# PierfrancescoArdino/C2M

Hardware: AMD Instinct MI355X
Metric: generator train-step frames/sec at 128x256x7 (higher is better)
Workload: dtype f32; 1 GPU; BASELINE configs[1]: 128x256, 7-frame clips (2 in + 5 predicted), batch 8/GPU, fp32, generator fwd+bwd only (no D), VGG loss on, random-init weights; global_batch=8, parallelism=single

## Files before the change

c2m_amd/csrc/conv_igemm.hip:

```cpp
#include "common.h"
#include "dtype.h"
#include <stdlib.h>
#include <string.h>
#include "conv_store.h"

typedef float f32x16 __attribute__((ext_vector_type(16)));
typedef float f32x4 __attribute__((ext_vector_type(4)));

struct ConvP {
    const float* A;
    const float* X;
    float* Y;
    const float* bias;
    const int4* ktab;
    int M, nk, lda;
    int Npix, To, Ho, Wo;
    int Ti, Hi, Wi;
    int st, sh, sw;
    int in_sc;
    long in_sn, in_st, in_sh;
    long out_sn, out_sc, out_st, out_sh, out_sw, out_off;
    long slab_stride;
    unsigned x_bytes;
    float* Y2;
// ... 935 lines not shown
        if (chunk < chunk_end) PB_CHUNK(s1);
    }
#undef PB_CHUNK
#undef PB_TAP

    const bool direct = blk.nz == 1;
    const bool yh = p.yh && direct;
    float* __restrict__ Yb = p.Y + (long)blk.z * p.slab_stride;
    if (yh && !p.Y2 && p.out_sw == 1 && (p.Wo & 7) == 0 && (p.out_off & 7) == 0 && (p.out_sc & 7) == 0 && (p.out_sn & 7) == 0 &&
        (p.out_st & 7) == 0 && (p.out_sh & 7) == 0 && ((uintptr_t)p.Y & 15) == 0 && BM >= 64) {
        float* __restrict__ T = reinterpret_cast<float*>(&sA[0][0]) + wave * (64 * 64);
        bf16_t* __restrict__ yimg = reinterpret_cast<bf16_t*>(p.Y) + p.out_off + (long)n_img * p.out_sn + (long)t_img * p.out_st;
#pragma unroll
        for (int h = 0; h < MI / 2; ++h) {
#pragma unroll
            for (int q = 0; q < 2; ++q)
#pragma unroll
                for (int jj = 0; jj < NI; ++jj)
#pragma unroll
                    for (int r = 0; r < 16; ++r) {
                        const int cl = q * 32 + (r & 3) + 8 * (r >> 2) + 4 * (lane >> 5);
                        float v = acc[2 * h + q][jj][r];
                        const int row = m0 + h * 64 + cl;
                        if (p.bias && row < p.M) v += p.bias[row];
                        T[cl * 64 + jj * 32 + (lane & 31)] = c2m_act(v, p.act, p.slope);
                    }
#pragma unroll
            for (int it = 0; it < 8; ++it) {
                const int cl = it * 8 + (lane >> 3), px = (lane & 7) * 8;
                const float4 v0 = *reinterpret_cast<const float4*>(&T[cl * 64 + px]);
                const float4 v1 = *reinterpret_cast<const float4*>(&T[cl * 64 + px + 4]);
                const int row = m0 + h * 64 + cl;
                const int oy = oy0 + wave * NI + (px >> 5), ox = ox0 + (px & 31);
                if (row < p.M && oy < p.Ho && ox < p.Wo) {
                    const bf16x8 o = {(bf16_t)v0.x, (bf16_t)v0.y, (bf16_t)v0.z, (bf16_t)v0.w,
                                      (bf16_t)v1.x, (bf16_t)v1.y, (bf16_t)v1.z, (bf16_t)v1.w};
                    __builtin_nontemporal_store(o, reinterpret_cast<bf16x8*>(yimg + (long)row * p.out_sc + (long)oy * p.out_sh + ox));
                }
            }
        }
        return;
    }
    if (!yh && !p.Y2 && p.out_sw == 1 && (p.Wo & 3) == 0 && (p.out_off & 3) == 0 && (p.out_sc & 3) == 0 && (p.out_sn & 3) == 0 &&
        (p.slab_stride & 3) == 0 && ((uintptr_t)p.Y & 15) == 0 && BM >= 64) {
        float* __restrict__ T = reinterpret_cast<float*>(&sA[0][0]) + wave * (64 * 64);
        float* __restrict__ yimg = Yb + p.out_off + (long)n_img * p.out_sn + (long)t_img * p.out_st;
#pragma unroll
        for (int h = 0; h < MI / 2; ++h) {
#pragma unroll
            for (int q = 0; q < 2; ++q)
#pragma unroll
                for (int jj = 0; jj < NI; ++jj)
#pragma unroll
                    for (int r = 0; r < 16; ++r) {
                        const int cl = q * 32 + (r & 3) + 8 * (r >> 2) + 4 * (lane >> 5);
                        float v = acc[2 * h + q][jj][r];
                        if (direct) {
                            const int row = m0 + h * 64 + cl;
                            if (p.bias && row < p.M) v += p.bias[row];
                            v = c2m_act(v, p.act, p.slope);
                        }
                        T[cl * 64 + jj * 32 + (lane & 31)] = v;
                    }
#pragma unroll
            for (int it = 0; it < 16; ++it) {
                const int cl = it * 4 + (lane >> 4), px = (lane & 15) * 4;
                const float4 v = *reinterpret_cast<const float4*>(&T[cl * 64 + px]);
                const int row = m0 + h * 64 + cl;
                const int oy = oy0 + wave * NI + (px >> 5), ox = ox0 + (px & 31);
                if (row < p.M && oy < p.Ho && ox < p.Wo) {
                    f32x4 vv = {v.x, v.y, v.z, v.w};
                    __builtin_nontemporal_store(vv, reinterpret_cast<f32x4*>(yimg + (long)row * p.out_sc + (long)oy * p.out_sh + ox));
                }
            }
        }
        return;
    }
#pragma unroll
    for (int j = 0; j < NI; ++j) {
        const int oy = oy0 + wave * NI + j, ox = ox0 + (lane & 31);
        if (oy >= p.Ho || ox >= p.Wo) continue;
        float* ybase = Yb;
        long yidx = p.out_off + (long)n_img * p.out_sn + (long)t_img * p.out_st + (long)oy * p.out_sh + (long)ox * p.out_sw;
        long row_stride = p.out_sc;
        if (p.Y2) {
            const int tp = t_img * p.ps_t + p.po_t - p.lo_t, yp = oy * p.ps_y + p.po_y - p.lo_y,
                      xp = ox * p.ps_x + p.po_x - p.lo_x;
            if ((unsigned)tp < (unsigned)p.ext_t && (unsigned)yp < (unsigned)p.ext_y && (unsigned)xp < (unsigned)p.ext_x) {
                ybase = p.Y2;
                yidx = (long)n_img * p.y2_sn + (long)tp * p.y2_st + (long)yp * p.y2_sh + xp;
                row_stride = p.y2_sc;
            }
        }
#pragma unroll
        for (int i = 0; i < MI; ++i)
#pragma unroll
            for (int r = 0; r < 16; ++r) {
                const int row = m0 + i * 32 + (r & 3) + 8 * (r >> 2) + 4 * (lane >> 5);
                if (row < p.M) {
                    float v = acc[i][j][r];
                    if (direct) {
                        if (p.bias) v += p.bias[row];
                        v = c2m_act(v, p.act, p.slope);
                    }
                    if (yh) reinterpret_cast<bf16_t*>(ybase)[yidx + (long)row * row_stride] = (bf16_t)v;
                    else ybase[yidx + (long)row * row_stride] = v;
                }
            }
    }
}

template <int BM>
static int launch_patch_bf16(const ConvP& p, int splits, hipStream_t s) {
    const long tiles = (long)(p.Npix / (p.Ho * p.Wo)) * ((p.Ho + 7) / 8) * ((p.Wo + 31) / 32);
    dim3 grid((unsigned)(tiles * c2m_cdiv(p.M, BM) * splits));
    hipLaunchKernelGGL((conv_patch3x3_bf16_kernel<BM>), grid, dim3(256), 0, s, p);
    return (int)hipGetLastError();
}

template <class T>
__global__ void splitk_reduce_kernel(const float* __restrict__ slab, T* __restrict__ out,
                                     const float* __restrict__ bias, long total, int S, long chan_stride, int M, int act,
                                     float slope) {
    for (long i = blockIdx.x * (long)blockDim.x + threadIdx.x; i < total; i += (long)gridDim.x * blockDim.x) {
        float acc = 0.f;
        for (int z = 0; z < S; ++z) acc += slab[(long)z * total + i];
        if (bias) acc += bias[(int)((i / chan_stride) % M)];
        c2m_st(out, i, c2m_act(acc, act, slope));
    }
}

template <typename I, class T = float>
__global__ void splitk_reduce_vec_kernel(const float4* __restrict__ slab, T* __restrict__ out,
                                         const float* __restrict__ bias, long total4_, int S, long chan_stride4_, int M,
                                         int act, float slope) {
    const I total4 = (I)total4_, chan_stride4 = (I)chan_stride4_;
    for (I i = blockIdx.x * (I)blockDim.x + threadIdx.x; i < total4; i += (I)gridDim.x * blockDim.x) {
        float4 acc = make_float4(0.f, 0.f, 0.f, 0.f);
        for (int z = 0; z < S; ++z) {
            const float4 v = slab[(long)z * total4_ + i];
            acc.x += v.x; acc.y += v.y; acc.z += v.z; acc.w += v.w;
        }
        if (bias) {
            const float b = bias[(int)((i / chan_stride4) % (I)M)];
            acc.x += b; acc.y += b; acc.z += b; acc.w += b;
        }
        c2m_st4(out + 4 * (long)i, make_float4(c2m_act(acc.x, act, slope), c2m_act(acc.y, act, slope), c2m_act(acc.z, act, slope),
                                               c2m_act(acc.w, act, slope)));
    }
}

template <int NS> static int launch_thin_fwd(const ConvP& p, hipStream_t s);
template <int KW> static int launch_thin_rows(const ConvP& p, int ns, int ntg, int Cin, int xdesc, hipStream_t s);

#ifndef C2M_IGEMM_U
#define C2M_IGEMM_U 1
#endif
#ifndef C2M_BF16_U
#define C2M_BF16_U 2
#endif

template <int BM, int BN, int WGM, int WGN>
static int launch_igemm(const ConvP& p, int ns, int splits, hipStream_t s, bool bf16) {
    dim3 grid((unsigned)c2m_cdiv(p.Npix, BN) * c2m_cdiv(p.M, BM) * splits * p.ncls);
    constexpr int U = (BM == 128) ? C2M_IGEMM_U : 1;
    if (bf16) {
        constexpr int UB = C2M_BF16_U;
        switch (ns) {
            case 1: hipLaunchKernelGGL((conv_igemm_kernel<BM, BN, WGM, WGN, 1, UB, true>), grid, dim3(256), 0, s, p); break;
            case 2: hipLaunchKernelGGL((conv_igemm_kernel<BM, BN, WGM, WGN, 2, UB, true>), grid, dim3(256), 0, s, p); break;
            case 4: hipLaunchKernelGGL((conv_igemm_kernel<BM, BN, WGM, WGN, 4, UB, true>), grid, dim3(256), 0, s, p); break;
            default: return (int)hipErrorInvalidValue;
        }
        return (int)hipGetLastError();
    }
    switch (ns) {
        case 1: hipLaunchKernelGGL((conv_igemm_kernel<BM, BN, WGM, WGN, 1, U>), grid, dim3(256), 0, s, p); break;
        case 2: hipLaunchKernelGGL((conv_igemm_kernel<BM, BN, WGM, WGN, 2, 1>), grid, dim3(256), 0, s, p); break;
        case 4: hipLaunchKernelGGL((conv_igemm_kernel<BM, BN, WGM, WGN, 4, 1>), grid, dim3(256), 0, s, p); break;
        default: return (int)hipErrorInvalidValue;
    }
    return (int)hipGetLastError();
}

static void igemm_tile(int M, int& BM, int& BN) {
    if (M <= 32) { BM = 32; BN = 256; }
    else if (M <= 64) { BM = 64; BN = 128; }
    else { BM = 128; BN = 128; }
}

C2M_API int c2m_conv_igemm_splits(int M, int nk, int Npix) {
    int BM, BN;
    igemm_tile(M, BM, BN);
    const long tiles = (long)c2m_cdiv(M, BM) * c2m_cdiv(Npix, BN);
#ifndef C2M_SPLIT_TARGET
#define C2M_SPLIT_TARGET 1280
#endif
    if (tiles >= 768 || nk < 8) return 1;
    long S = (C2M_SPLIT_TARGET + tiles - 1) / tiles;
    if (S > nk / 4) S = nk / 4;
    if (S > 128) S = 128;
    if (S < 2) return 1;
    const int per = c2m_cdiv(nk, (int)S);
    return c2m_cdiv(nk, per);
}

C2M_API int c2m_conv_igemm(const float* A, const void* X, void* Y, void* Y_interior, const float* bias,
                           const int* ktab, const int64_t* g, int act, float slope, void* stream) {
    C2M_ENTER();
    ConvP p;
    p.A = A; p.X = (const float*)X; p.Y = (float*)Y; p.bias = bias; p.ktab = reinterpret_cast<const int4*>(ktab);
    p.Y2 = (float*)Y_interior;
    p.ps_t = (int)g[C2M_G_PS_T]; p.ps_y = (int)g[C2M_G_PS_Y]; p.ps_x = (int)g[C2M_G_PS_X]; p.po_t = (int)g[C2M_G_PO_T]; p.po_y = (int)g[C2M_G_PO_Y];
    p.po_x = (int)g[C2M_G_PO_X]; p.lo_t = (int)g[C2M_G_LO_T]; p.lo_y = (int)g[C2M_G_LO_Y]; p.lo_x = (int)g[C2M_G_LO_X]; p.ext_t = (int)g[C2M_G_EXT_T];
    p.ext_y = (int)g[C2M_G_EXT_Y]; p.ext_x = (int)g[C2M_G_EXT_X]; p.y2_sn = g[C2M_G_Y2_SN]; p.y2_sc = g[C2M_G_Y2_SC]; p.y2_st = g[C2M_G_Y2_ST]; p.y2_sh = g[C2M_G_Y2_SH];
    p.M = (int)g[C2M_G_M]; p.nk = (int)g[C2M_G_NK]; p.lda = (int)g[C2M_G_LDA];
    p.Npix = (int)g[C2M_G_NPIX]; p.To = (int)g[C2M_G_TO]; p.Ho = (int)g[C2M_G_HO]; p.Wo = (int)g[C2M_G_WO];
    p.Ti = (int)g[C2M_G_TI]; p.Hi = (int)g[C2M_G_HI]; p.Wi = (int)g[C2M_G_WI];
    p.st = (int)g[C2M_G_ST]; p.sh = (int)g[C2M_G_SH]; p.sw = (int)g[C2M_G_SW];
    p.in_sn = g[C2M_G_IN_SN]; p.in_st = g[C2M_G_IN_ST]; p.in_sh = g[C2M_G_IN_SH];
    p.out_sn = g[C2M_G_OUT_SN]; p.out_sc = g[C2M_G_OUT_SC]; p.out_st = g[C2M_G_OUT_ST]; p.out_sh = g[C2M_G_OUT_SH]; p.out_sw = g[C2M_G_OUT_SW]; p.out_off = g[C2M_G_OUT_OFF];
    p.reflect = (int)g[C2M_G_REFLECT]; p.is3d = (int)g[C2M_G_IS3D];
    const int ns = (int)g[C2M_G_NS];
    p.in_sc = (int)g[C2M_G_IN_SC];
    const int splits = (int)g[C2M_G_SPLITS];
    p.slab_stride = g[C2M_G_SLAB_STRIDE];
    if (g[C2M_G_X_BYTES] <= 0 || g[C2M_G_X_BYTES] >= 0x80000000LL) return (int)hipErrorInvalidValue;
    p.x_bytes = (unsigned)g[C2M_G_X_BYTES];
    p.act = act; p.slope = slope;
    p.xh = (int)g[C2M_G_X_TYPE]; p.yh = (int)g[C2M_G_Y_TYPE];
    if ((p.xh | p.yh) & ~1) return (int)hipErrorInvalidValue;
    if (p.M <= 0 || p.Npix <= 0) return 0;
    if (p.nk <= 0 || (p.lda & 3) || (((uintptr_t)A) & 15) || splits < 1) return (int)hipErrorInvalidValue;
    if (p.Y2 && splits != 1) return (int)hipErrorInvalidValue;
    p.ksteps_per_split = c2m_cdiv(p.nk, splits);
    if (!g[C2M_G_PATCH] && c2m_cdiv(p.nk, p.ksteps_per_split) != splits) return (int)hipErrorInvalidValue;
    p.splits = splits;
    p.ncls = g[C2M_G_NCLS] > 1 ? (int)g[C2M_G_NCLS] : 1;
    if (p.ncls > 8) return (int)hipErrorInvalidValue;
    p.a_cls = g[C2M_G_A_CLS]; p.ktab_cls = (int)g[C2M_G_KTAB_CLS];
    p.out_off_c[0] = p.out_off; p.po_c[0][0] = p.po_t; p.po_c[0][1] = p.po_y; p.po_c[0][2] = p.po_x;
    for (int c = 0; c < p.ncls && p.ncls > 1; ++c) {
        p.out_off_c[c] = g[C2M_G_CLS_OUT_OFF + c];
        for (int d = 0; d < 3; ++d) p.po_c[c][d] = (int)g[C2M_G_CLS_PO + 3 * c + d];
    }
    if (p.ncls > 1 && (g[C2M_G_PATCH] || (p.a_cls & 3))) return (int)hipErrorInvalidValue;
    hipStream_t s = (hipStream_t)stream;
    if (g[C2M_G_G8] == 1) {
        const int C = (int)g[C2M_G_CIN], taps = (int)g[C2M_G_TAPS];
        if (g[C2M_G_PRECISION] != 1 || !p.xh || g[C2M_G_PATCH] || C <= 0 || taps <= 0 || taps > 64 || (((uintptr_t)A | (uintptr_t)X) & 15))
            return (int)hipErrorInvalidValue;
        p.g8_nch = c2m_cdiv(C, 16); p.g8_ntaps = taps; p.g8_CB = c2m_cdiv(C, 8); p.g8_Mpad = c2m_cdiv(p.M, 128) * 128;
        if (p.nk != taps * p.g8_nch || p.in_st != (long)p.Hi * p.Wi || p.in_sh != p.Wi) return (int)hipErrorInvalidValue;
        const long plane = (long)p.Ti * p.Hi * p.Wi * 16, ab = (long)p.nk * 2 * p.g8_Mpad * 16;
        if (plane * p.g8_CB > (long)p.x_bytes || p.x_bytes % (plane * p.g8_CB) || ab * p.ncls >= 0x80000000LL)
            return (int)hipErrorInvalidValue;
        p.g8_plane_bytes = (unsigned)plane; p.g8_a_bytes = (unsigned)ab;
        const unsigned ptiles = (unsigned)c2m_cdiv(p.Npix, 256);
        int v = (int)g[C2M_G_G8_VARIANT] & 255;
        p.g8_dbg = (int)(g[C2M_G_G8_VARIANT] >> 8);
        if (v == 0) v = p.M <= 32 ? 1 : ((p.M <= 64 || (p.M % 128 >= 1 && p.M % 128 <= 64)) ? 5 : 3);
#define G8_LAUNCH(BM, UU, NB, WG) do {                                                                                     \
            dim3 grid(ptiles * (unsigned)c2m_cdiv(p.M, BM) * (unsigned)(splits * p.ncls));                                  \
            hipLaunchKernelGGL((conv_gather_nc8_kernel<BM, UU, NB, WG>), grid, dim3(256), 0, s, p); } while (0)
        switch (v) {
            case 1: G8_LAUNCH(32, 4, 2, 2); break;
            case 2: G8_LAUNCH(64, 2, 3, 2); break;
            case 3: G8_LAUNCH(128, 2, 3, 2); break;
            case 4: G8_LAUNCH(64, 1, 4, 3); break;
            case 5: G8_LAUNCH(64, 2, 2, 3); break;
            case 6: G8_LAUNCH(128, 1, 4, 2); break;
            case 7: G8_LAUNCH(32, 2, 3, 2); break;
            default: return (int)hipErrorInvalidValue;
        }
#undef G8_LAUNCH
        return (int)hipGetLastError();
    }
    if (g[C2M_G_PATCH]) {
        if (ns != 1 || p.st != 1 || p.sh != 1 || p.sw != 1) return (int)hipErrorInvalidValue;
        p.iy0 = (int)g[C2M_G_PATCH_IY0]; p.ix0 = (int)g[C2M_G_PATCH_IX0];
        for (int i = 0; i < 3; ++i) { p.pty[i] = (int)g[C2M_G_PATCH_TY + i]; p.ptx[i] = (int)g[C2M_G_PATCH_TX + i]; }
        p.nchunks = p.nk / 9;
        p.cin = (int)g[C2M_G_CIN];
        if (p.nchunks * 9 != p.nk || p.cin <= 0 || p.cin > p.nchunks * 16) return (int)hipErrorInvalidValue;
        p.ksteps_per_split = c2m_cdiv(p.nchunks, splits);
        if (c2m_cdiv(p.nchunks, p.ksteps_per_split) != splits) return (int)hipErrorInvalidValue;
        if (g[C2M_G_PRECISION] == 1) {
            if (p.lda % 128 != 0 || p.lda < p.M || !p.xh) return (int)hipErrorInvalidValue;
            if (p.M <= 32)      return launch_patch_bf16<32>(p, splits, s);
            else if (p.M <= 64 || p.cin <= 256) return launch_patch_bf16<64>(p, splits, s);
            else                return launch_patch_bf16<128>(p, splits, s);
        }
        if (p.xh || p.yh) return (int)hipErrorInvalidValue;
        if (p.M <= 32)      return launch_patch<32, 256, 1, 4>(p, splits, s);
        else if (p.M <= 64) return launch_patch<64, 128, 2, 2>(p, splits, s);
        else                return launch_patch<128, 128, 2, 2>(p, splits, s);
    }
    if (p.M <= 4 && splits == 1 && p.Npix >= 16384 && !p.Y2 && p.ncls == 1) {
        if (p.xh || p.yh) return (int)hipErrorInvalidValue;
        const int kw = (int)(g[C2M_G_SQUARE_KW] < 0 ? -g[C2M_G_SQUARE_KW] : g[C2M_G_SQUARE_KW]);
        if (p.M <= 3 && (kw == 3 || kw == 7) && !p.is3d && p.To == 1 && p.st == 1 && p.sh == 1 && p.sw == 1 && p.Wo % 4 == 0 &&
            g[C2M_G_TAPS] == kw * kw && g[C2M_G_CIN] > 0 && g[C2M_G_CIN] * kw * kw * 16 <= 48 * 1024) {
            if (kw == 3) return launch_thin_rows<3>(p, ns, (int)g[C2M_G_NTG], (int)g[C2M_G_CIN], g[C2M_G_SQUARE_KW] < 0, s);
            return launch_thin_rows<7>(p, ns, (int)g[C2M_G_NTG], (int)g[C2M_G_CIN], g[C2M_G_SQUARE_KW] < 0, s);
        }
        if (ns == 1) return launch_thin_fwd<1>(p, s);
        if (ns == 2) return launch_thin_fwd<2>(p, s);
        return launch_thin_fwd<4>(p, s);
    }
    const bool bf16 = g[C2M_G_PRECISION] == 1;
    if (bf16 ? !p.xh : (p.xh || p.yh)) return (int)hipErrorInvalidValue;
    if (p.M <= 32)      return launch_igemm<32, 256, 1, 4>(p, ns, splits, s, bf16);
    else if (p.M <= 64) return launch_igemm<64, 128, 2, 2>(p, ns, splits, s, bf16);
    else                return launch_igemm<128, 128, 2, 2>(p, ns, splits, s, bf16);
}

C2M_API int c2m_splitk_reduce(const float* slab, void* out, const float* bias, long total, int splits,
                              long chan_stride, int M, int act, float slope, int dt, void* stream) {
    C2M_ENTER();
    if (total <= 0) return 0;
    const uintptr_t omask = dt == C2M_BF16 ? 7 : 15;
    const bool vec = (total & 3) == 0 && (!bias || (chan_stride & 3) == 0) && (((uintptr_t)slab) & 15) == 0 &&
                     (((uintptr_t)out) & omask) == 0;
    const dim3 grid(c2m_grid(vec ? total / 4 : total, 256));
    hipStream_t s = (hipStream_t)stream;
    C2M_DISPATCH_DT(dt,
        if (vec) {
            if (total / 4 < (1L << 31))
                hipLaunchKernelGGL((splitk_reduce_vec_kernel<unsigned, T>), grid, dim3(256), 0, s, reinterpret_cast<const float4*>(slab),
                                   (T*)out, bias, total / 4, splits, bias ? chan_stride / 4 : 1, M, act, slope);
            else
                hipLaunchKernelGGL((splitk_reduce_vec_kernel<long, T>), grid, dim3(256), 0, s, reinterpret_cast<const float4*>(slab),
                                   (T*)out, bias, total / 4, splits, bias ? chan_stride / 4 : 1, M, act, slope);
        } else {
            hipLaunchKernelGGL(splitk_reduce_kernel<T>, grid, dim3(256), 0, s, slab, (T*)out, bias, total, splits, chan_stride, M,
                               act, slope);
        });
    return (int)hipGetLastError();
}

struct WgradP {
    const float* dY;
    const float* X;
    float* slab;
    const int4* jtab;
    int M, J;
    int Npix, To, Ho, Wo, Ti, Hi, Wi, st, sh, sw;
    int in_sc;
    long in_sn, in_st, in_sh;
    long dy_sn, dy_sc;
    int pix_per_split;
    int reflect, is3d;
    unsigned x_bytes, dy_bytes;
};

template <int BM, int BN, int WGM, int WGN, int NS, bool BF = false>
__global__ __launch_bounds__(256) void conv_wgrad_kernel(const WgradP p) {
    constexpr int CK = 16 / NS;
    constexpr int BK = 64;
    constexpr int LDS_S = BK + 1;
    constexpr int TM = BM / WGM, TN = BN / WGN, MI = TM / 32, NI = TN / 32;
    constexpr int AROWS = BM / 4, BROWSW = BN / 4;
    constexpr int BGROUPS = BROWSW / 16;
    static_assert(BROWSW % 16 == 0, "wgrad rows per wave must be whole tap groups");
    constexpr int LDH = BK + 8;
    __shared__ float sA[BF ? 1 : BM][BF ? 1 : LDS_S];
    __shared__ float sB[BF ? 1 : BN][BF ? 1 : LDS_S];
    __shared__ __attribute__((aligned(16))) __bf16 hA[BF ? BM : 1][BF ? LDH : 8];
    __shared__ __attribute__((aligned(16))) __bf16 hB[BF ? BN : 1][BF ? LDH : 8];
    const int tid = threadIdx.x, lane = tid & 63;
    const int wave = __builtin_amdgcn_readfirstlane(tid >> 6);
    const int wm = wave / WGN, wn = wave % WGN;
    const C2mBlock blk = c2m_xcd_block((unsigned)p.J / BN, (unsigned)(p.M + BM - 1) / BM, 0);
    const int m0 = blk.y * BM, j0 = blk.x * BN;
    const int split = blk.z;
    const int pbeg = split * p.pix_per_split;
    int pend = pbeg + p.pix_per_split; pend = pend < p.Npix ? pend : p.Npix;
    const int in_st = (int)p.in_st, in_sh = (int)p.in_sh;

    f32x16 acc[MI][NI];
#pragma unroll
    for (int i = 0; i < MI; ++i)
#pragma unroll
        for (int j = 0; j < NI; ++j)
#pragma unroll
            for (int r = 0; r < 16; ++r) acc[i][j][r] = 0.f;

    float ra[AROWS], rb[BROWSW];
    constexpr int XES = BF ? 2 : 4;
    auto ldv = [&](const __amdgpu_buffer_rsrc_t& rs, unsigned vo, int soff_elems) -> float {
        if constexpr (BF) return __uint_as_float((unsigned)__builtin_amdgcn_raw_buffer_load_b16(rs, vo, soff_elems * 2, 0) << 16);
        else return __builtin_bit_cast(float, __builtin_amdgcn_raw_buffer_load_b32(rs, vo, soff_elems * 4, 0));
    };
    const __amdgpu_buffer_rsrc_t yrsrc = __builtin_amdgcn_make_buffer_rsrc(const_cast<float*>(p.dY), 0, p.dy_bytes, 0x00020000);
    const __amdgpu_buffer_rsrc_t xrsrc = __builtin_amdgcn_make_buffer_rsrc(const_cast<float*>(p.X), 0, p.x_bytes, 0x00020000);
    auto issue_loads = [&](int pk) {
        const int pix = pk + lane;
        const bool live = pix < pend;
        int n, ot, oy, ox;
        decompose_pix(live ? pix : pend - 1, p, n, ot, oy, ox);
        const int sp = (ot * p.Ho + oy) * p.Wo + ox;
        const unsigned yvo = live ? (unsigned)(n * (int)p.dy_sn + sp) * (unsigned)XES : C2M_OOB;
        const unsigned ximg = (unsigned)(n * (int)p.in_sn) * (unsigned)XES;
        const int ots = ot * p.st, oys = oy * p.sh, oxs = ox * p.sw;
#pragma unroll
        for (int s = 0; s < AROWS; ++s) {
            const int row = m0 + wave * AROWS + s;
            ra[s] = ldv(yrsrc, yvo, row * (int)p.dy_sc);
        }
#pragma unroll
        for (int gq = 0; gq < BGROUPS; ++gq) {
            const int grp = (j0 + wave * BROWSW) / 16 + gq;
            const int4* __restrict__ jd = p.jtab + (long)grp * (1 + NS);
            const int4 hdr = jd[0];
            unsigned vo[NS];
#pragma unroll
            for (int q = 0; q < NS; ++q) {
                const int so = spatial_off(jd[1 + q], ots, oys, oxs, p.Ti, p.Hi, p.Wi, in_st, in_sh, p.reflect, p.is3d);
                vo[q] = (live && so >= 0) ? ximg + (unsigned)so * (unsigned)XES : C2M_OOB;
            }
            if (hdr.y == -2) {
#pragma unroll
                for (int s = 0; s < 16; ++s) rb[gq * 16 + s] = (s == 0) ? 1.f : 0.f;
            } else {
#pragma unroll
                for (int s = 0; s < 16; ++s) {
                    const int slot = s / CK, cc = s % CK;
                    rb[gq * 16 + s] = ldv(xrsrc, vo[slot], hdr.x + cc * p.in_sc);
                }
            }
        }
    };
    struct PixCtx { unsigned yvo, ximg; int ots, oys, oxs; bool live; };
    auto load_prep = [&](int pk) {
        const int pix = pk + lane;
        PixCtx c;
        c.live = pix < pend;
        int n, ot, oy, ox;
        decompose_pix(c.live ? pix : pend - 1, p, n, ot, oy, ox);
        const int sp = (ot * p.Ho + oy) * p.Wo + ox;
        c.yvo = c.live ? (unsigned)(n * (int)p.dy_sn + sp) * (unsigned)XES : C2M_OOB;
        c.ximg = (unsigned)(n * (int)p.in_sn) * (unsigned)XES;
        c.ots = ot * p.st; c.oys = oy * p.sh; c.oxs = ox * p.sw;
        return c;
    };
    auto load_a_part = [&](const PixCtx& c, int s0, int s1) {
#pragma unroll
        for (int s = s0; s < s1; ++s) {
            const int row = m0 + wave * AROWS + s;
            ra[s] = ldv(yrsrc, c.yvo, row * (int)p.dy_sc);
        }
    };
    auto load_b_group = [&](const PixCtx& c, int gq) {
        const int grp = (j0 + wave * BROWSW) / 16 + gq;
        const int4* __restrict__ jd = p.jtab + (long)grp * (1 + NS);
// ... 416 lines not shown
        for (int kt = 0; kt < p.nk; ++kt) {
            const int4* __restrict__ kd = p.ktab + (long)kt * (1 + NS);
            const int4 hdr = kd[0];
            unsigned vo[NS];
#pragma unroll
            for (int q = 0; q < NS; ++q) {
                const int so = spatial_off(kd[1 + q], ots, oys, oxs, p.Ti, p.Hi, p.Wi, in_st, in_sh, p.reflect, p.is3d);
                vo[q] = so >= 0 ? img_byte + (unsigned)so * 4u : C2M_OOB;
            }
            float xv[16];
#pragma unroll
            for (int e = 0; e < 16; ++e)
                xv[e] = __builtin_bit_cast(float, __builtin_amdgcn_raw_buffer_load_b32(
                    xrsrc, vo[e / CK], (hdr.x + (e % CK) * p.in_sc) * 4, 0));
#pragma unroll
            for (int m = 0; m < MT; ++m) {
                const float* __restrict__ wr = p.A + (long)m * p.lda + kt * 16;
#pragma unroll
                for (int e = 0; e < 16; ++e) acc[m] = fmaf(xv[e], wr[e], acc[m]);
            }
        }
        float* __restrict__ yb = p.Y + p.out_off + (long)n * p.out_sn + (long)ot * p.out_st + (long)oy * p.out_sh +
                                 (long)ox * p.out_sw;
#pragma unroll
        for (int m = 0; m < MT; ++m) {
            if (m < p.M) {
                float v = acc[m];
                if (p.bias) v += p.bias[m];
                yb[(long)m * p.out_sc] = c2m_act(v, p.act, p.slope);
            }
        }
    }
}

template <int MT, int KW>
__global__ __launch_bounds__(256) void conv_thin_rows_kernel(const ConvP p, int lns, int ntg, int Cin, int xdesc) {
    constexpr int PX = 4, NV = PX + KW - 1;
    extern __shared__ float4 sW[];
    const int NS = 1 << lns, CK = 16 >> lns, lck = 4 - lns;
    auto tap_entry = [&](int t) { return p.ktab[(t >> lns) * (1 + NS) + 1 + (t & (NS - 1))]; };
    for (int e = threadIdx.x; e < Cin * KW * KW; e += 256) {
        const int c = e / (KW * KW), t = e - c * (KW * KW);
        const int k = (((c >> lck) * ntg + (t >> lns)) << 4) + ((t & (NS - 1)) << lck) + (c & (CK - 1));
        float w[4] = {0.f, 0.f, 0.f, 0.f};
#pragma unroll
        for (int m = 0; m < MT; ++m) w[m] = p.A[(long)m * p.lda + k];
        sW[e] = make_float4(w[0], w[1], w[2], w[3]);
    }
    __syncthreads();
    const __amdgpu_buffer_rsrc_t xrsrc = __builtin_amdgcn_make_buffer_rsrc(const_cast<float*>(p.X), 0, p.x_bytes, 0x00020000);
    const int groups_x = p.Wo / PX;
    const int total = p.Npix / PX;
    const int dx_first = tap_entry(0).z, dx_last = tap_entry(KW - 1).z;
    const int lo = dx_first < dx_last ? dx_first : dx_last;
    constexpr int HL = (KW - 1) / 2;
    const bool sym = lo == -HL && p.Wi == p.Wo && (p.in_sh % 4) == 0 && (p.in_sc % 4) == 0 && (p.in_sn % 4) == 0 &&
                     (((uintptr_t)p.X) & 15) == 0;
    const int lane = threadIdx.x & 63;
    const int rounds = (total - (int)blockIdx.x * 256 + (int)gridDim.x * 256 - 1) / ((int)gridDim.x * 256);
    int g = blockIdx.x * 256 + threadIdx.x;
    for (int it = 0; it < rounds; ++it, g += gridDim.x * 256) {
        const bool live = g < total;
        const int gg = live ? g : total - 1;
        const int xg = gg % groups_x; int r = gg / groups_x;
        const int oy = r % p.Ho; const int n = r / p.Ho;
        const int ox0 = xg * PX;
        const unsigned img_byte = (unsigned)(n * (int)p.in_sn) * 4u;
        float acc[MT][PX];
#pragma unroll
        for (int m = 0; m < MT; ++m)
#pragma unroll
            for (int q = 0; q < PX; ++q) acc[m][q] = 0.f;
        const bool first = xg == 0, last = xg == groups_x - 1;
        const bool memL = live && !first && lane == 0;
        const bool memR = live && !last && (lane == 63 || g + 1 >= total);
        unsigned cvo[NV];
#pragma unroll
        for (int e = 0; e < NV; ++e) {
            int ix = ox0 + lo + e;
            bool ok = live;
            if (p.reflect) { ix = ix < 0 ? -ix : ix; ix = ix >= p.Wi ? 2 * p.Wi - 2 - ix : ix; }
            else ok = ok && (unsigned)ix < (unsigned)p.Wi;
            cvo[e] = ok ? (unsigned)ix * 4u : C2M_OOB;
        }
        for (int i = 0; i < KW; ++i) {
            int iy = oy + tap_entry(i * KW).y;
            bool rok = live;
            if (p.reflect) { iy = iy < 0 ? -iy : iy; iy = iy >= p.Hi ? 2 * p.Hi - 2 - iy : iy; }
            else rok = rok && (unsigned)iy < (unsigned)p.Hi;
            const unsigned rbase = img_byte + (unsigned)(iy * (int)p.in_sh) * 4u;
            unsigned vo[NV];
#pragma unroll
            for (int e = 0; e < NV; ++e) vo[e] = (rok && cvo[e] != C2M_OOB) ? rbase + cvo[e] : C2M_OOB;
            const unsigned own_vo = rok ? rbase + (unsigned)ox0 * 4u : C2M_OOB;
            const float4* __restrict__ wrow = sW + i * KW;
            for (int c = 0; c < Cin; ++c) {
                float v[NV];
                if (sym) {
                    const int soff = c * p.in_sc * 4;
                    const f32x4 own = __builtin_bit_cast(f32x4, __builtin_amdgcn_raw_buffer_load_b128(xrsrc, own_vo, soff, 0));
                    v[HL + 0] = own.x; v[HL + 1] = own.y; v[HL + 2] = own.z; v[HL + 3] = own.w;
#pragma unroll
                    for (int e = 0; e < HL; ++e) {
                        const float ml = __builtin_bit_cast(float, __builtin_amdgcn_raw_buffer_load_b32(
                            xrsrc, (rok && memL) ? own_vo - (unsigned)(HL - e) * 4u : C2M_OOB, soff, 0));
                        const float mr = __builtin_bit_cast(float, __builtin_amdgcn_raw_buffer_load_b32(
                            xrsrc, (rok && memR) ? own_vo + (unsigned)(4 + e) * 4u : C2M_OOB, soff, 0));
                        const float up = __shfl_up(v[4 + e], 1, 64);
                        const float dn = __shfl_down(v[HL + e], 1, 64);
                        const float bl = p.reflect ? v[HL + HL - e] : 0.f;
                        const float br = p.reflect ? v[HL + 2 - e] : 0.f;
                        v[e] = memL ? ml : (first ? bl : up);
                        v[HL + 4 + e] = memR ? mr : (last ? br : dn);
                    }
                } else {
#pragma unroll
                    for (int e = 0; e < NV; ++e)
                        v[e] = __builtin_bit_cast(float, __builtin_amdgcn_raw_buffer_load_b32(xrsrc, vo[e], c * p.in_sc * 4, 0));
                }
#pragma unroll
                for (int j = 0; j < KW; ++j) {
                    const float4 w4 = wrow[c * (KW * KW) + j];
                    const float wv[4] = {w4.x, w4.y, w4.z, w4.w};
                    const int pos = xdesc ? KW - 1 - j : j;
#pragma unroll
                    for (int m = 0; m < MT; ++m)
#pragma unroll
                        for (int q = 0; q < PX; ++q) acc[m][q] = fmaf(v[q + pos], wv[m], acc[m][q]);
                }
            }
        }
        if (!live) continue;
        float* __restrict__ yb = p.Y + p.out_off + (long)n * p.out_sn + (long)oy * p.out_sh + (long)ox0 * p.out_sw;
#pragma unroll
        for (int m = 0; m < MT; ++m) {
            if (m < p.M) {
                float o[PX];
#pragma unroll
                for (int q = 0; q < PX; ++q) {
                    float v = acc[m][q];
                    if (p.bias) v += p.bias[m];
                    o[q] = c2m_act(v, p.act, p.slope);
                }
                float* dst = yb + (long)m * p.out_sc;
                if (p.out_sw == 1 && (((uintptr_t)dst) & 15) == 0) {
                    *reinterpret_cast<float4*>(dst) = make_float4(o[0], o[1], o[2], o[3]);
                } else {
#pragma unroll
                    for (int q = 0; q < PX; ++q) dst[(long)q * p.out_sw] = o[q];
                }
            }
        }
    }
}

template <int KW>
static int launch_thin_rows(const ConvP& p, int ns, int ntg, int Cin, int xdesc, hipStream_t s) {
    long blocks = (p.Npix / 4 + 255) / 256;
    if (blocks > 2048) blocks = 2048;
    dim3 grid((unsigned)blocks);
    const int lns = ns == 1 ? 0 : (ns == 2 ? 1 : 2);
    const size_t lds = (size_t)Cin * KW * KW * sizeof(float4);
    switch (p.M) {
        case 1: hipLaunchKernelGGL((conv_thin_rows_kernel<1, KW>), grid, dim3(256), lds, s, p, lns, ntg, Cin, xdesc); break;
        case 2: hipLaunchKernelGGL((conv_thin_rows_kernel<2, KW>), grid, dim3(256), lds, s, p, lns, ntg, Cin, xdesc); break;
        case 3: hipLaunchKernelGGL((conv_thin_rows_kernel<3, KW>), grid, dim3(256), lds, s, p, lns, ntg, Cin, xdesc); break;
        default: hipLaunchKernelGGL((conv_thin_rows_kernel<4, KW>), grid, dim3(256), lds, s, p, lns, ntg, Cin, xdesc); break;
    }
    return (int)hipGetLastError();
}

template <int NS>
static int launch_thin_fwd(const ConvP& p, hipStream_t s) {
    dim3 grid(c2m_grid(p.Npix, 256));
    switch (p.M) {
        case 1: hipLaunchKernelGGL((conv_thin_fwd_kernel<1, NS>), grid, dim3(256), 0, s, p); break;
        case 2: hipLaunchKernelGGL((conv_thin_fwd_kernel<2, NS>), grid, dim3(256), 0, s, p); break;
        case 3: hipLaunchKernelGGL((conv_thin_fwd_kernel<3, NS>), grid, dim3(256), 0, s, p); break;
        default: hipLaunchKernelGGL((conv_thin_fwd_kernel<4, NS>), grid, dim3(256), 0, s, p); break;
    }
    return (int)hipGetLastError();
}

template <int MT, int NS, int GPB>
__global__ __launch_bounds__(256) void conv_thin_wgrad_kernel(const WgradP p, int ngroups_total) {
    constexpr int CK = 16 / NS;
    __shared__ float red[4][GPB * 16 * MT];
    const int lane = threadIdx.x & 63, wave = threadIdx.x >> 6;
    const int g0 = blockIdx.x * GPB;
    const int split = blockIdx.z;
    const int pbeg = split * p.pix_per_split;
    int pend = pbeg + p.pix_per_split; pend = pend < p.Npix ? pend : p.Npix;
    const int in_st = (int)p.in_st, in_sh = (int)p.in_sh;
    const __amdgpu_buffer_rsrc_t xrsrc = __builtin_amdgcn_make_buffer_rsrc(const_cast<float*>(p.X), 0, p.x_bytes, 0x00020000);
    float acc[GPB][16][MT];
#pragma unroll
    for (int g = 0; g < GPB; ++g)
#pragma unroll
        for (int s = 0; s < 16; ++s)
#pragma unroll
            for (int m = 0; m < MT; ++m) acc[g][s][m] = 0.f;
    for (int pix = pbeg + threadIdx.x; pix < pend; pix += 256) {
        int n, ot, oy, ox;
        decompose_pix(pix, p, n, ot, oy, ox);
        const int sp = (ot * p.Ho + oy) * p.Wo + ox;
        float dy[MT];
#pragma unroll
        for (int m = 0; m < MT; ++m) dy[m] = m < p.M ? p.dY[(long)n * p.dy_sn + (long)m * p.dy_sc + sp] : 0.f;
        const unsigned ximg = (unsigned)(n * (int)p.in_sn) * 4u;
        const int ots = ot * p.st, oys = oy * p.sh, oxs = ox * p.sw;
#pragma unroll
        for (int g = 0; g < GPB; ++g) {
            const int grp = g0 + g;
            if (grp >= ngroups_total) break;
            const int4* __restrict__ jd = p.jtab + (long)grp * (1 + NS);
            const int4 hdr = jd[0];
            if (hdr.y == -2) {
#pragma unroll
                for (int m = 0; m < MT; ++m) acc[g][0][m] += dy[m];
                continue;
            }
            unsigned vo[NS];
#pragma unroll
            for (int q = 0; q < NS; ++q) {
                const int so = spatial_off(jd[1 + q], ots, oys, oxs, p.Ti, p.Hi, p.Wi, in_st, in_sh, p.reflect, p.is3d);
                vo[q] = so >= 0 ? ximg + (unsigned)so * 4u : C2M_OOB;
            }
#pragma unroll
            for (int s = 0; s < 16; ++s) {
                const float x = __builtin_bit_cast(float, __builtin_amdgcn_raw_buffer_load_b32(
                    xrsrc, vo[s / CK], (hdr.x + (s % CK) * p.in_sc) * 4, 0));
#pragma unroll
                for (int m = 0; m < MT; ++m) acc[g][s][m] = fmaf(dy[m], x, acc[g][s][m]);
            }
        }
    }
#pragma unroll
    for (int g = 0; g < GPB; ++g)
#pragma unroll
        for (int s = 0; s < 16; ++s)
#pragma unroll
            for (int m = 0; m < MT; ++m) {
                const float v = wave_sum(acc[g][s][m]);
                if (lane == 0) red[wave][(g * 16 + s) * MT + m] = v;
            }
    __syncthreads();
    float* __restrict__ out = p.slab + (long)split * p.M * p.J;
    for (int i = threadIdx.x; i < GPB * 16 * MT; i += 256) {
        const int m = i % MT, gs = i / MT;
        const int col = g0 * 16 + gs;
        if (m < p.M && col < ngroups_total * 16)
            out[(long)m * p.J + col] = (red[0][i] + red[1][i]) + (red[2][i] + red[3][i]);
    }
}

template <int MT, int KW, int CPB, int RI>
__global__ __launch_bounds__(256) void conv_thin_wgrad_rows_kernel(const WgradP p, int lns, int ntg, int Cin, int ngroups,
                                                                   int quads_per_split) {
    constexpr int PX = 4, NV = PX + KW - 1, NACC = CPB * RI * KW * MT;
    __shared__ float red[4][NACC + MT];
    const int NS = 1 << lns, lck = 4 - lns, CK = 16 >> lns;
    const int lane = threadIdx.x & 63, wave = threadIdx.x >> 6;
    const int c0 = blockIdx.x * CPB;
    const int i0 = blockIdx.y * RI;
    const int split = blockIdx.z;
    const int groups_x = p.Wo / PX;
    const int total = p.Npix / PX;
    const int qbeg = split * quads_per_split;
    int qend = qbeg + quads_per_split; qend = qend < total ? qend : total;
    auto tap_entry = [&](int t) { return p.jtab[(t >> lns) * (1 + NS) + 1 + (t & (NS - 1))]; };
    const int dx0 = tap_entry(0).z, dy0 = tap_entry(0).y;
    const __amdgpu_buffer_rsrc_t xrsrc = __builtin_amdgcn_make_buffer_rsrc(const_cast<float*>(p.X), 0, p.x_bytes, 0x00020000);
    float acc[CPB][RI][KW][MT];
    float accb[MT];
#pragma unroll
    for (int c = 0; c < CPB; ++c)
#pragma unroll
        for (int i = 0; i < RI; ++i)
#pragma unroll
            for (int j = 0; j < KW; ++j)
#pragma unroll
                for (int m = 0; m < MT; ++m) acc[c][i][j][m] = 0.f;
#pragma unroll
    for (int m = 0; m < MT; ++m) accb[m] = 0.f;
    constexpr int HL = (KW - 1) / 2;
    auto load_group = [&](int g, float (&dy)[MT][PX], float (&v)[RI][CPB][NV], int& fl) {
        const bool live = g < qend;
        const int gg = live ? g : qend - 1;
        const int xg = gg % groups_x; const int r = gg / groups_x;
        const int oy = r % p.Ho; const int n = r / p.Ho;
        const int ox0 = xg * PX;
        const bool first = xg == 0, last = xg == groups_x - 1;
        const bool memL = live && !first && lane == 0;
        const bool memR = live && !last && (lane == 63 || g + 1 >= qend);
        fl = (first ? 2 : 0) | (last ? 4 : 0) | (memL ? 8 : 0) | (memR ? 16 : 0);
#pragma unroll
        for (int m = 0; m < MT; ++m) {
            if (m < p.M && live) {
                const float4 t = *reinterpret_cast<const float4*>(p.dY + (long)n * p.dy_sn + (long)m * p.dy_sc + (long)oy * p.Wo + ox0);
                dy[m][0] = t.x; dy[m][1] = t.y; dy[m][2] = t.z; dy[m][3] = t.w;
            } else {
#pragma unroll
                for (int q = 0; q < PX; ++q) dy[m][q] = 0.f;
            }
        }
        const unsigned img_byte = (unsigned)(n * (int)p.in_sn) * 4u;
// ... 702 lines not shown
```

Measured before the change: 895.0 frames/s.

## Add 2D LDS-tiled thin-output conv kernel with double-buffered channel prefetch

Adds a new kernel for thin-output (M<=3) 3x3 and 7x7 stride-1 convolutions. Each block stages a 64-wide by 16*R-tall input tile plus halo for one channel at a time in LDS, double-buffered, and prefetches the next channel through buffer loads while computing. Each thread produces R rows of 4 pixels, so the halo is shared and redundant global reads are removed compared with the per-row kernel. Dispatch uses it when the input is aligned and the LDS budget fits, which adds another code path and adds LDS pressure that can limit occupancy.

New measurement: 903.6 frames/s (median of 6 runs). No clear change (+1.0%).

```diff
diff --git a/c2m_amd/csrc/conv_igemm.hip b/c2m_amd/csrc/conv_igemm.hip
--- a/c2m_amd/csrc/conv_igemm.hip
+++ b/c2m_amd/csrc/conv_igemm.hip
@@ -1111,6 +1111,14 @@
 
 template <int NS> static int launch_thin_fwd(const ConvP& p, hipStream_t s);
 template <int KW> static int launch_thin_rows(const ConvP& p, int ns, int ntg, int Cin, int xdesc, hipStream_t s);
+#ifndef C2M_THIN_TILE_R7
+#define C2M_THIN_TILE_R7 2
+#endif
+#ifndef C2M_THIN_TILE_R3
+#define C2M_THIN_TILE_R3 2
+#endif
+template <int KW, int R> static int launch_thin_tile(const ConvP& p, int ns, int ntg, int Cin, hipStream_t s);
+template <int KW, int R> static size_t thin_tile_lds(int Cin);
 
 #ifndef C2M_IGEMM_U
 #define C2M_IGEMM_U 1
@@ -1260,6 +1268,12 @@
         const int kw = (int)(g[C2M_G_SQUARE_KW] < 0 ? -g[C2M_G_SQUARE_KW] : g[C2M_G_SQUARE_KW]);
         if (p.M <= 3 && (kw == 3 || kw == 7) && !p.is3d && p.To == 1 && p.st == 1 && p.sh == 1 && p.sw == 1 && p.Wo % 4 == 0 &&
             g[C2M_G_TAPS] == kw * kw && g[C2M_G_CIN] > 0 && g[C2M_G_CIN] * kw * kw * 16 <= 48 * 1024) {
+            const int cin = (int)g[C2M_G_CIN];
+            const bool aligned = p.Wi == p.Wo && (p.in_sh % 4) == 0 && (p.in_sc % 4) == 0 && (p.in_sn % 4) == 0 && (((uintptr_t)p.X) & 15) == 0;
+            if (aligned && kw == 3 && thin_tile_lds<3, C2M_THIN_TILE_R3>(cin) <= 64 * 1024)
+                return launch_thin_tile<3, C2M_THIN_TILE_R3>(p, ns, (int)g[C2M_G_NTG], cin, s);
+            if (aligned && kw == 7 && thin_tile_lds<7, C2M_THIN_TILE_R7>(cin) <= 64 * 1024)
+                return launch_thin_tile<7, C2M_THIN_TILE_R7>(p, ns, (int)g[C2M_G_NTG], cin, s);
             if (kw == 3) return launch_thin_rows<3>(p, ns, (int)g[C2M_G_NTG], (int)g[C2M_G_CIN], g[C2M_G_SQUARE_KW] < 0, s);
             return launch_thin_rows<7>(p, ns, (int)g[C2M_G_NTG], (int)g[C2M_G_CIN], g[C2M_G_SQUARE_KW] < 0, s);
         }
@@ -1982,6 +1996,152 @@
             }
         }
     }
+}
+
+template <int MT, int KW, int R>
+__global__ __launch_bounds__(256) void conv_thin_tile_kernel(const ConvP p, int lns, int ntg, int Cin, int tiles_x, int tiles_y) {
+    constexpr int KK = KW * KW, TW = 64, TH = 16 * R, TIW = TW + KW - 1, TIH = TH + KW - 1, LS = 72;
+    constexpr int NV4 = (4 + KW - 1 + 3) / 4, NL = (TIH * TIW + 255) / 256, UD = KW == 7 ? 1 : KW;
+    static_assert(60 + NV4 * 4 <= LS, "window reads stay inside an LDS row");
+    extern __shared__ float4 sW[];
+    float* __restrict__ sX = reinterpret_cast<float*>(sW + Cin * KK);
+    const int NS = 1 << lns, CK = 16 >> lns, lck = 4 - lns;
+    auto tap_entry = [&](int t) { return p.ktab[(t >> lns) * (1 + NS) + 1 + (t & (NS - 1))]; };
+    const int4 t00 = tap_entry(0), t0e = tap_entry(KW - 1), tee = tap_entry(KK - 1);
+    const int lo_x = t00.z < t0e.z ? t00.z : t0e.z, lo_y = t00.y < tee.y ? t00.y : tee.y;
+    for (int e = threadIdx.x; e < Cin * KK; e += 256) {
+        const int c = e / KK, t = e - c * KK;
+        const int k = (((c >> lck) * ntg + (t >> lns)) << 4) + ((t & (NS - 1)) << lck) + (c & (CK - 1));
+        float w[4] = {0.f, 0.f, 0.f, 0.f};
+#pragma unroll
+        for (int m = 0; m < MT; ++m) w[m] = p.A[(long)m * p.lda + k];
+        const int4 tp = tap_entry(t);
+        const int d = tp.y - lo_y, pos = tp.z - lo_x;
+        if ((unsigned)d < (unsigned)KW && (unsigned)pos < (unsigned)KW) sW[c * KK + d * KW + pos] = make_float4(w[0], w[1], w[2], w[3]);
+    }
+    const __amdgpu_buffer_rsrc_t xrsrc = __builtin_amdgcn_make_buffer_rsrc(const_cast<float*>(p.X), 0, p.x_bytes, 0x00020000);
+    const int tx = blockIdx.x % tiles_x; int rb = blockIdx.x / tiles_x;
+    const int ty = rb % tiles_y; const int n = rb / tiles_y;
+    const int ox_t = tx * TW, oy_t = ty * TH;
+    const unsigned img_byte = (unsigned)(n * (int)p.in_sn) * 4u;
+    unsigned svo[NL];
+    int sld[NL];
+#pragma unroll
+    for (int k = 0; k < NL; ++k) {
+        const int e = threadIdx.x + k * 256;
+        const int row = e / TIW, col = e - row * TIW;
+        int iy = oy_t + lo_y + row, ix = ox_t + lo_x + col;
+        if (p.reflect) {
+            iy = iy < 0 ? -iy : iy; iy = iy >= p.Hi ? 2 * p.Hi - 2 - iy : iy;
+            ix = ix < 0 ? -ix : ix; ix = ix >= p.Wi ? 2 * p.Wi - 2 - ix : ix;
+        }
+        const bool in_tile = row < TIH;
+        const bool ok = in_tile && (unsigned)iy < (unsigned)p.Hi && (unsigned)ix < (unsigned)p.Wi;
+        svo[k] = ok ? img_byte + (unsigned)(iy * (int)p.in_sh + ix) * 4u : C2M_OOB;
+        sld[k] = in_tile ? row * LS + col : -1;
+    }
+    float pre[NL];
+#pragma unroll
+    for (int k = 0; k < NL; ++k) pre[k] = __builtin_bit_cast(float, __builtin_amdgcn_raw_buffer_load_b32(xrsrc, svo[k], 0, 0));
+#pragma unroll
+    for (int k = 0; k < NL; ++k) if (sld[k] >= 0) sX[sld[k]] = pre[k];
+    __syncthreads();
+    const int xq = threadIdx.x & 15, ly = threadIdx.x >> 4;
+    float acc[R][MT][4];
+#pragma unroll
+    for (int r = 0; r < R; ++r)
+#pragma unroll
+        for (int m = 0; m < MT; ++m)
+#pragma unroll
+            for (int q = 0; q < 4; ++q) acc[r][m][q] = 0.f;
+    for (int c = 0; c < Cin; ++c) {
+        const float* __restrict__ buf = sX + (c & 1) * (TIH * LS);
+        const bool more = c + 1 < Cin;
+        if (more) {
+            const int soff = (c + 1) * p.in_sc * 4;
+#pragma unroll
+            for (int k = 0; k < NL; ++k) pre[k] = __builtin_bit_cast(float, __builtin_amdgcn_raw_buffer_load_b32(xrsrc, svo[k], soff, 0));
+        }
+        const float4* __restrict__ wc = sW + c * KK;
+        const float* __restrict__ win = buf + (ly * R) * LS + 4 * xq;
+#pragma unroll UD
+        for (int d = 0; d < KW; ++d) {
+            float v[R][NV4 * 4];
+#pragma unroll
+            for (int r = 0; r < R; ++r) {
+                const float4* __restrict__ src = reinterpret_cast<const float4*>(win + (d + r) * LS);
+#pragma unroll
+                for (int h = 0; h < NV4; ++h) {
+                    const float4 t4 = src[h];
+                    v[r][4 * h] = t4.x; v[r][4 * h + 1] = t4.y; v[r][4 * h + 2] = t4.z; v[r][4 * h + 3] = t4.w;
+                }
+            }
+#pragma unroll
+            for (int pos = 0; pos < KW; ++pos) {
+                const float4 w4 = wc[d * KW + pos];
+                const float wv[4] = {w4.x, w4.y, w4.z, w4.w};
+#pragma unroll
+                for (int r = 0; r < R; ++r)
+#pragma unroll
+                    for (int m = 0; m < MT; ++m)
+#pragma unroll
+                        for (int q = 0; q < 4; ++q) acc[r][m][q] = fmaf(v[r][q + pos], wv[m], acc[r][m][q]);
+            }
+        }
+        if (more) {
+            float* __restrict__ nb = sX + ((c + 1) & 1) * (TIH * LS);
+#pragma unroll
+            for (int k = 0; k < NL; ++k) if (sld[k] >= 0) nb[sld[k]] = pre[k];
+        }
+        __syncthreads();
+    }
+    const int ox0 = ox_t + 4 * xq;
+    if (ox0 >= p.Wo) return;
+#pragma unroll
+    for (int r = 0; r < R; ++r) {
+        const int oy = oy_t + ly * R + r;
+        if (oy >= p.Ho) continue;
+        float* __restrict__ yb = p.Y + p.out_off + (long)n * p.out_sn + (long)oy * p.out_sh + (long)ox0 * p.out_sw;
+#pragma unroll
+        for (int m = 0; m < MT; ++m) {
+            if (m < p.M) {
+                float o[4];
+#pragma unroll
+                for (int q = 0; q < 4; ++q) {
+                    float a = acc[r][m][q];
+                    if (p.bias) a += p.bias[m];
+                    o[q] = c2m_act(a, p.act, p.slope);
+                }
+                float* dst = yb + (long)m * p.out_sc;
+                if (p.out_sw == 1 && (((uintptr_t)dst) & 15) == 0) {
+                    *reinterpret_cast<float4*>(dst) = make_float4(o[0], o[1], o[2], o[3]);
+                } else {
+#pragma unroll
+                    for (int q = 0; q < 4; ++q) dst[(long)q * p.out_sw] = o[q];
+                }
+            }
+        }
+    }
+}
+
+template <int KW, int R>
+static size_t thin_tile_lds(int Cin) {
+    return (size_t)Cin * KW * KW * sizeof(float4) + 2 * (size_t)(16 * R + KW - 1) * 72 * sizeof(float);
+}
+
+template <int KW, int R>
+static int launch_thin_tile(const ConvP& p, int ns, int ntg, int Cin, hipStream_t s) {
+    const int tiles_x = c2m_cdiv(p.Wo, 64), tiles_y = c2m_cdiv(p.Ho, 16 * R), nimg = p.Npix / (p.Ho * p.Wo);
+    dim3 grid((unsigned)tiles_x * tiles_y * nimg);
+    const int lns = ns == 1 ? 0 : (ns == 2 ? 1 : 2);
+    const size_t lds = thin_tile_lds<KW, R>(Cin);
+    switch (p.M) {
+        case 1: hipLaunchKernelGGL((conv_thin_tile_kernel<1, KW, R>), grid, dim3(256), lds, s, p, lns, ntg, Cin, tiles_x, tiles_y); break;
+        case 2: hipLaunchKernelGGL((conv_thin_tile_kernel<2, KW, R>), grid, dim3(256), lds, s, p, lns, ntg, Cin, tiles_x, tiles_y); break;
+        case 3: hipLaunchKernelGGL((conv_thin_tile_kernel<3, KW, R>), grid, dim3(256), lds, s, p, lns, ntg, Cin, tiles_x, tiles_y); break;
+        default: return (int)hipErrorInvalidValue;
+    }
+    return (int)hipGetLastError();
 }
 
 template <int KW>
```
